# theOehrly/Formula-VAD

Measured on AMD Instinct MI355X. Metric: 48 kHz 480-sample VAD frames/sec whole node; max concurrent real-time streams, higher is better.
Workload: dtype f32

## Files before the change

### formula-vad_amd/csrc/fvad_vadm.hip

```cpp
#pragma clang fp contract(off)
#include <hip/hip_runtime.h>

#include "fvad_device.h"
#include "fvad_exact.h"
#include "fvad_internal.h"
#include "fvad_launch.h"
#include "fvad_staged.h"
#include "fvad_staged_dev.h"
#include "fvad_vadm_dev.h"

namespace fvad {

__device__ void vadm_stream(const StagedArgs &a, int m, int s, float *lt, size_t lts, bool final) {
  const int B = a.n_streams, C = a.n_channels, nb = a.n_bands;
  const int nt = ticks_of(a, s);
  const VadmConst &K = a.vadm.c[m];
  VadmState S = a.vadm.st[(size_t)m * B + s];
  float *st = a.vadm.buf + K.st_off + s, *rb = a.vadm.buf + K.r_off + s;
  VadmSeg *seg = a.vadm.seg + ((size_t)m * B + s) * a.vadm.seg_cap;
  const VadmEvLane ev = vadm_ev_lane(a.vadm, m, s);
  vadm_walk(S, K, st, rb, B, lt, lts, seg, a.vadm.seg_cap, ev, (unsigned long long)a.plan->nfft_b,
            a.vadm.bound_scale, a.vadm.defer_max, a.vadm.count, final, [&](auto &&window) {
              for (int t = 0; t < nt; t++)
                for (int w = 0, nw = a.out_win_flag[(size_t)t * B + s]; w < nw; w++) {
                  const size_t o = ((size_t)t * B + s) * a.wpt + w;
                  float min_v = 999, max_v = 0;
                  for (int c = 0; c < C; c++) {
                    const float v = a.out_band[(o * C + c) * nb + K.slot];
                    if (v < min_v) min_v = v;
                    if (v > max_v) max_v = v;
                  }
                  if ((long long)S.windows_done == a.vadm.negate_at) min_v = -min_v;
                  window(min_v, a.use_denoiser ? a.out_win_vad[o] : 0.0f, a.out_win_ratio[o]);
                }
            });
  a.vadm.st[(size_t)m * B + s] = S;
}

#ifndef FVAD_VP_BLOCK
#define FVAD_VP_BLOCK 8
#endif
constexpr int kVpG = 16, kVpS = 4, kVpMaxW = 48;
__device__ __forceinline__ double lt_fold(double acc, const float *lt, size_t lts, unsigned i0, unsigned i1, unsigned nw,
                                          double init, double scalar) {
  if (i0 >= i1) return acc;
  return lt_range<FVAD_VP_BLOCK>(acc, lt, lts, i0, i1, nw, init, scalar);
}
__global__ void __launch_bounds__(64) k_vadm_par(StagedArgs a) {
  __shared__ float wmin[kVpS][kVpMaxW], wvad[kVpS][kVpMaxW], wvr[kVpS][kVpMaxW];
  __shared__ float pv[kVpS][kVpMaxW];
  __shared__ double favg[kVpS][kVpG];
  __shared__ double rpre[kVpS];
  __shared__ int rnd[kVpS][4];
  __shared__ VadmState Ss[kVpS];
  const int B = a.n_streams, C = a.n_channels, nb = a.n_bands;
  const int g = threadIdx.x / kVpG, r = threadIdx.x % kVpG;
  const int s = blockIdx.x * kVpS + g;
  const bool sok = s < B && ticks_of(a, s) > 0;
  const int nt = sok ? ticks_of(a, s) : 0;
  const unsigned long long fft = (unsigned long long)a.plan->nfft_b;
  const int self = threadIdx.x;
  for (int m = 0; m < a.vadm.n; m++) {
    const VadmConst &K = a.vadm.c[m];
    float *lt = a.vadm.buf + K.lt_off + (size_t)(sok ? s : 0) * K.lt_pitch;
    const size_t lts = 1;
    int Kw = 0;
    for (int t0 = 0; t0 < nt; t0 += kVpG) {
      const int t = t0 + r;
      const int nwt = t < nt ? a.out_win_flag[(size_t)t * B + s] : 0;
      int pos = nwt;
#pragma unroll
      for (int d = 1; d < kVpG; d <<= 1) {
        const int up = __shfl(pos, self - d);
        if (r >= d) pos += up;
      }
      const int tot = __shfl(pos, g * kVpG + kVpG - 1);
      for (int w = 0; w < nwt; w++) {
        const int k = Kw + pos - nwt + w;
        if (k < kVpMaxW) {
          const size_t o = ((size_t)t * B + s) * a.wpt + w;
          float min_v = 999;
          for (int c = 0; c < C; c++) {
            const float v = a.out_band[(o * C + c) * nb + K.slot];
            if (v < min_v) min_v = v;
          }
          wmin[g][k] = min_v;
          wvad[g][k] = a.use_denoiser ? a.out_win_vad[o] : 0.0f;
          wvr[g][k] = a.out_win_ratio[o];
        }
      }
      Kw += tot;
    }
    if (r == 0) {
      Ss[g] = a.vadm.st[(size_t)m * B + (sok ? s : 0)];
      if (sok) {
        lt_resolve(Ss[g], K, lt, lts);
      } else if (s < B) {
        VadmState S2 = a.vadm.st[(size_t)m * B + s];
        if (S2.lt_defer) {
          lt_resolve(S2, K, a.vadm.buf + K.lt_off + (size_t)s * K.lt_pitch, 1);
          a.vadm.st[(size_t)m * B + s] = S2;
        }
      }
    }
    wave_sync();
    if (r == 0 && sok && a.vadm.negate_at >= 0) {
      const long long k = a.vadm.negate_at - (long long)Ss[g].windows_done;
      if (k >= 0 && k < Kw && k < kVpMaxW) wmin[g][k] = -wmin[g][k];
      wave_sync();
    }
    VadmState &S = Ss[g];
    float *st = a.vadm.buf + K.st_off + (sok ? s : 0), *rb = a.vadm.buf + K.r_off + (sok ? s : 0);
    VadmSeg *seg = a.vadm.seg + ((size_t)m * B + (sok ? s : 0)) * a.vadm.seg_cap;
    const VadmEvLane ev = vadm_ev_lane(a.vadm, m, sok ? s : 0);
    const bool forced = a.vadm.par_serial_every > 0 && s % a.vadm.par_serial_every == 0;
    const bool fast = sok && !forced && Kw <= kVpMaxW && K.n_lt > kVpMaxW && S.lt_count == (unsigned)K.n_lt &&
                      S.lt_pre_ok;
    const unsigned n = (unsigned)K.n_lt, wbase = S.lt_widx, nw0 = S.lt_nw;
    const double scalar = 1.0 / (double)n;
    if (r == 0) {
      rnd[g][0] = 0;
      rnd[g][1] = 0;
      rnd[g][2] = !sok ? 1 : (fast ? 0 : 2);
    }
    wave_sync();
    int j = 0, npush = 0;
    double pre = S.lt_pre;
    for (;;) {
      if (r == 0 && rnd[g][2] == 0) {
        while (j < Kw) {
          const unsigned long long index = S.windows_done * fft;
          const bool met = vadm_short(S, K, st, rb, B, wmin[g][j], wvr[g][j]);
          if (!met) break;
          S.windows_done++;
          vadm_fsm(S, K, index, met, wvad[g][j], wvr[g][j], seg, a.vadm.seg_cap, ev);
          j++;
        }
        if (j >= Kw) rnd[g][2] = 1;
        rnd[g][0] = j;
        rnd[g][1] = npush;
        for (int q = 0; q < kVpG && j + q < Kw; q++) pv[g][npush + q] = wmin[g][j + q];
        rpre[g] = pre;
      }
      wave_sync();
      const int state = rnd[g][2];
      if (__ballot(state == 0) == 0) break;
      if (state == 0) {
        const int j0 = rnd[g][0], np = rnd[g][1];
        if (j0 + r < Kw) {
          const unsigned k = (unsigned)(np + r);
          const unsigned nw = min(n, nw0 + k + 1);
          double P = rpre[g];
          unsigned w = (wbase + (unsigned)np) % n;
#pragma unroll 1
          for (int q = 0; q < r; q++) {
            P = (w + 1 == n) ? 0.0 : P + (double)pv[g][np + q] * scalar;
            w = (w + 1 == n) ? 0u : w + 1;
          }
          double acc = P + (double)pv[g][np + r] * scalar;
          if (wbase + k < n) {
            acc = lt_fold(acc, lt, lts, w + 1, n, nw, K.init, scalar);
          } else {
            acc = lt_fold(acc, lt, lts, w + 1, wbase, nw, K.init, scalar);
            for (unsigned i = wbase; i < n; i++) acc += (double)pv[g][i - wbase] * scalar;
          }
          favg[g][r] = acc;
        }
      }
      wave_sync();
      if (r == 0 && state == 0) {
        const int j0 = j;
        for (int q = 0; q < kVpG && j0 + q < Kw; q++) {
          const int jj = j0 + q;
          const unsigned long long index = S.windows_done * fft;
          bool met = false;
          if (q > 0) met = vadm_short(S, K, st, rb, B, wmin[g][jj], wvr[g][jj]);
          if (!met) {
            const unsigned w = S.lt_widx;
            S.lt_widx = (w + 1) % n;
            if (S.lt_nw < n) S.lt_nw++;
            pre = (w + 1 == n) ? 0.0 : pre + (double)wmin[g][jj] * scalar;
            S.lt_pre = pre;
            S.lt_last = favg[g][q];
            S.lt_has = 1;
            lt_neg_push(S, n, wmin[g][jj]);
            npush++;
          }
          S.windows_done++;
          vadm_fsm(S, K, index, met, wvad[g][jj], wvr[g][jj], seg, a.vadm.seg_cap, ev);
          j = jj + 1;
          if (met) break;
        }
      }
      wave_sync();
    }
    if (r == 0 && sok) {
      if (rnd[g][2] == 2) {
        vadm_stream(a, m, s, lt, lts, true);
      } else {
        unsigned w = wbase;
#pragma unroll 1
        for (int q = 0; q < npush; q++) {
          lt[(size_t)w * lts] = pv[g][q];
          w = (w + 1 == n) ? 0u : w + 1;
        }
        a.vadm.st[(size_t)m * B + s] = S;
      }
    }
    wave_sync();
  }
}

#ifndef FVAD_VADM_LANES
#define FVAD_VADM_LANES 64
#endif
constexpr int kVadmHbmLanes = FVAD_VADM_LANES;
__global__ void __launch_bounds__(64) k_vadm_hbm(StagedArgs a) {
  const int s = blockIdx.x * blockDim.x + threadIdx.x;
  if (s >= a.n_streams) return;
  const bool final = a.vadm.vfinal != 0;
  if (ticks_of(a, s) <= 0) {
    if (final)
      for (int m = 0; m < a.vadm.n; m++) {
        VadmState *p = a.vadm.st + (size_t)m * a.n_streams + s;
        if (p->lt_defer) {
          VadmState S = *p;
          lt_resolve(S, a.vadm.c[m], a.vadm.buf + a.vadm.c[m].lt_off + (size_t)s * a.vadm.c[m].lt_pitch, 1);
          *p = S;
        }
      }
    return;
  }
  for (int m = 0; m < a.vadm.n; m++)
    vadm_stream(a, m, s, a.vadm.buf + a.vadm.c[m].lt_off + (size_t)s * a.vadm.c[m].lt_pitch, 1, final);
}

hipError_t launch_vadm(const StagedArgs &a, hipStream_t stream, bool fast, bool *ran_par) {
  (void)hipGetLastError();
  bool par = fast && a.wmax <= kVpMaxW;
  for (int m = 0; m < a.vadm.n; m++) par = par && a.vadm.c[m].has_init && a.vadm.c[m].n_lt > kVpMaxW;
  if (ran_par) *ran_par = par;
  if (!par)
    FVAD_KERNEL_TRY(k_vadm_hbm, dim3((a.n_streams + kVadmHbmLanes - 1) / kVadmHbmLanes), dim3(kVadmHbmLanes), 0,
                    stream, a);
  else
    FVAD_KERNEL_TRY(k_vadm_par, dim3((a.n_streams + kVpS - 1) / kVpS), dim3(kVpS * kVpG), 0, stream, a);
  return hipSuccess;
}

constexpr int kEvThreads = 256;
__global__ void __launch_bounds__(kEvThreads) k_vadm_events(VadmEventArgs a) {
  __shared__ unsigned wsum[kEvThreads / 64];
  const int tid = threadIdx.x, wl = tid & 63, wave = tid >> 6;
  const unsigned long long wr0 = a.cursor[0];
  const unsigned long long used = wr0 - a.host_read;
  const unsigned long long room = used < a.ring_cap ? a.ring_cap - used : 0ull;
  const int chunk = a.chunk > 0 && a.chunk < kEvThreads ? a.chunk : kEvThreads;
  unsigned long long base = 0;
  for (int l0 = 0; l0 < a.n_lanes; l0 += chunk) {
    const int l = l0 + tid;
    const bool on = tid < chunk && l < a.n_lanes;
    const unsigned c = on ? min(a.count[l], (unsigned)a.ev_cap) : 0u;
    unsigned inc = c;
#pragma unroll
    for (int d = 1; d < 64; d <<= 1) {
      const unsigned up = __shfl_up(inc, d);
      if (wl >= d) inc += up;
    }
    if (wl == 63) wsum[wave] = inc;
    __syncthreads();
    unsigned before = 0, total = 0;
#pragma unroll
    for (int w = 0; w < kEvThreads / 64; w++) {
      const unsigned v = wsum[w];
      if (w < wave) before += v;
      total += v;
    }
    const unsigned long long first = base + before + (inc - c);
    for (unsigned j = 0; j < c; j++) {
      const unsigned long long pos = first + j;
      if (pos >= room) break;
      const VadmEvRec r = a.stage[(size_t)l * a.ev_cap + j];
      VadmEvent e;
      e.kind = r.kind;
      e.stream = l / a.n_machines;
      e.machine = l % a.n_machines;
      e.seq = r.seq;
      e.push = a.push;
      e.sample_from = r.sample_from;
      e.sample_to = r.sample_to;
      e.debug_rnn_vad = r.debug_rnn_vad;
      e.debug_avg_speech_vol_ratio = r.debug_avg_speech_vol_ratio;
      a.ring[(wr0 + pos) % a.ring_cap] = e;
    }
    if (c) a.count[l] = 0;
    base += total;
    __syncthreads();
  }
  if (tid == 0) {
    const unsigned long long written = base < room ? base : room;
    const unsigned long long lost = a.cursor[1] + (base - written);
    a.cursor[0] = wr0 + written;
    a.cursor[1] = lost;
    VadmEventHeader h;
    h.pass = a.pass;
    h.end = wr0 + written;
    h.lost = lost;
    h.n = base;
    *a.header = h;
  }
}

hipError_t launch_vadm_events(const VadmEventArgs &a, hipStream_t stream) {
  (void)hipGetLastError();
  FVAD_KERNEL_TRY(k_vadm_events, dim3(1), dim3(kEvThreads), 0, stream, a);
  return hipSuccess;
}

constexpr int kSelStreams = 4;
#ifndef FVAD_SEL_RING
#define FVAD_SEL_RING 8
#endif
constexpr int kSelRing = FVAD_SEL_RING;
struct SelRec {
  int T0, nv, Tk, offk, off0;
  float g0, xy0, yy0, gk, xyk, yyk;
};
__device__ __forceinline__ void sel_load(SelRec &r, const float *__restrict__ row, int k, bool on) {
  if (!on) return;
  r.T0 = __float_as_int(row[rec::kT0]);
  r.nv = __float_as_int(row[rec::kNValid]);
  r.g0 = row[rec::kG0];
  r.xy0 = row[rec::kXy0];
  r.yy0 = row[rec::kYy0];
  r.off0 = __float_as_int(row[rec::kOff0]);
  const float *q = row + rec::kK + min(k, 13) * rec::kKStride;
  r.Tk = __float_as_int(q[0]);
  r.gk = q[1];
  r.xyk = q[2];
  r.yyk = q[3];
  r.offk = __float_as_int(q[4]);
}

__global__ void __launch_bounds__(64) k_select(StagedArgs a) {
  const int lane = threadIdx.x, sl = lane >> 4, k = lane & 15;
  static_assert(kWorkSlots * kQueues <= 64, "one lane per counter");
  if (blockIdx.x == 0 && lane < kWorkSlots * kQueues) a.work[lane] = 0;
  const int s = blockIdx.x * kSelStreams + sl;
  const bool sok = s < a.n_streams;
  const int nf = sok ? ticks_of(a, s) * a.n_channels : 0;
  int nfw = nf;
#pragma unroll
  for (int d = 16; d < 64; d <<= 1) nfw = max(nfw, __shfl_xor(nfw, d));
  if (nfw <= 0) return;
  float *stp = a.state + (size_t)(sok ? s : 0) * st::kWords;
  int *istp = reinterpret_cast<int *>(stp);
  int last_period = sok ? istp[st::kLastPeriod] : 0;
  float last_gain = sok ? stp[st::kLastGain] : 0.0f;
  const float *rows = a.rec + (size_t)(sok ? s : 0) * a.V * rec::kSize;
  const int K = k + 2;
  auto step = [&](const SelRec &r, int v) {
    const bool on = v < nf;
    const int prev_period = last_period / 2;
    const float prev_gain = last_gain;
    bool pass = false;
    if (on && k < 14 && k < r.nv) {
      const int T1 = r.Tk;
      float cont;
      if (abs(T1 - prev_period) <= 1)
        cont = prev_gain;
      else if (abs(T1 - prev_period) <= 2 && 5 * K * K < r.T0)
        cont = .5f * prev_gain;
      else
        cont = 0;
      float thresh;
      {
        const float vv = .7f * r.g0 - cont;
        thresh = (.3f > vv) ? .3f : vv;
      }
      if (T1 < 3 * 30) {
        const float vv = .85f * r.g0 - cont;
        thresh = (.4f > vv) ? .4f : vv;
      } else if (T1 < 2 * 30) {
        const float vv = .9f * r.g0 - cont;
        thresh = (.5f > vv) ? .5f : vv;
      }
      pass = r.gk > thresh;
    }
    const unsigned seg = (unsigned)(__ballot(pass) >> (16 * sl)) & 0x3fffu;
    const int win = seg ? 31 - __clz(seg) : 0;
    const int src = 16 * sl + win;
    const float wxy = __shfl(r.xyk, src), wyy = __shfl(r.yyk, src), wg = __shfl(r.gk, src);
    const int wT = __shfl(r.Tk, src), woff = __shfl(r.offk, src);
    float best_xy = seg ? wxy : r.xy0, best_yy = seg ? wyy : r.yy0, gg = seg ? wg : r.g0;
    const int T = seg ? wT : r.T0, offset = seg ? woff : r.off0;
    if (!on) return;
    best_xy = (0 > best_xy) ? 0 : best_xy;
    float pg;
    if (best_yy <= best_xy)
      pg = 1.0f;
    else
      pg = best_xy / (best_yy + 1);
    if (pg > gg) pg = gg;
    int pi = 2 * T + offset;
    if (pi < kPitchMin) pi = kPitchMin;
    if (k == 0) a.pitch[(size_t)s * a.V + v] = pi;
    last_period = pi;
    last_gain = pg;
  };
  SelRec r[kSelRing];
#pragma unroll
  for (int u = 0; u < kSelRing - 1; u++) {
    r[u] = SelRec{};
    sel_load(r[u], rows + (size_t)u * rec::kSize, k, u < nf);
  }
  r[kSelRing - 1] = SelRec{};
  for (int v = 0; v < nfw; v += kSelRing) {
#pragma unroll
    for (int u = 0; u < kSelRing; u++) {
      if (v + u >= nfw) break;
      const int ls = (u + kSelRing - 1) % kSelRing;
      sel_load(r[ls], rows + (size_t)(v + u + kSelRing - 1) * rec::kSize, k, v + u + kSelRing - 1 < nf);
      step(r[u], v + u);
    }
  }
  if (sok && nf > 0 && k == 0) {
    istp[st::kLastPeriod] = last_period;
    stp[st::kLastGain] = last_gain;
  }
}

hipError_t launch_select(const StagedArgs &a, hipStream_t stream) {
  FVAD_KERNEL_TRY(k_select, dim3((a.n_streams + kSelStreams - 1) / kSelStreams), dim3(64), 0, stream, a);
  return hipSuccess;
}

}
```

Baseline: 45.27 million.

## Precompute per-candidate select terms ahead and cut k_select's serial dependency chain

Restructures k_select so the work that does not depend on the previous frame's pitch (pg, pi, threshold base/floor, live mask) is computed a few frames ahead in sel_prep. The serial step is reduced to one ballot plus two ds_bpermute lookups. Records are loaded with vector memcpy and clamped indices instead of predicated scalar loads. Pitch outputs are buffered per lane and written once per ring pass instead of one lane storing every frame. This shortens the loop-carried latency chain at the cost of more registers for the ring of prepared options.

```diff
diff --git a/formula-vad_amd/csrc/fvad_vadm.hip b/formula-vad_amd/csrc/fvad_vadm.hip
--- a/formula-vad_amd/csrc/fvad_vadm.hip
+++ b/formula-vad_amd/csrc/fvad_vadm.hip
@@ -321,29 +321,76 @@
 #ifndef FVAD_SEL_RING
 #define FVAD_SEL_RING 8
 #endif
+#ifndef FVAD_SEL_AHEAD
+#define FVAD_SEL_AHEAD 2
+#endif
 constexpr int kSelRing = FVAD_SEL_RING;
+constexpr int kSelAhead = FVAD_SEL_AHEAD;
+static_assert(kSelRing <= 16 && kSelAhead >= 1 && kSelAhead <= kSelRing - 2, "k_select's ring");
+typedef float SelF4 __attribute__((ext_vector_type(4)));
+typedef float SelF2 __attribute__((ext_vector_type(2)));
 struct SelRec {
-  int T0, nv, Tk, offk, off0;
-  float g0, xy0, yy0, gk, xyk, yyk;
+  SelF4 sh;
+  SelF2 sh2;
+  SelF4 c;
+  float coff;
 };
-__device__ __forceinline__ void sel_load(SelRec &r, const float *__restrict__ row, int k, bool on) {
-  if (!on) return;
-  r.T0 = __float_as_int(row[rec::kT0]);
-  r.nv = __float_as_int(row[rec::kNValid]);
-  r.g0 = row[rec::kG0];
-  r.xy0 = row[rec::kXy0];
-  r.yy0 = row[rec::kYy0];
-  r.off0 = __float_as_int(row[rec::kOff0]);
-  const float *q = row + rec::kK + min(k, 13) * rec::kKStride;
-  r.Tk = __float_as_int(q[0]);
-  r.gk = q[1];
-  r.xyk = q[2];
-  r.yyk = q[3];
-  r.offk = __float_as_int(q[4]);
+struct SelOpt {
+  int T1, pi;
+  float g1, base, floor, pg;
+  bool near2;
+  unsigned long long live;
+};
+static_assert(rec::kT0 == 0 && rec::kNValid == 1 && rec::kG0 == 2 && rec::kXy0 == 3 && rec::kYy0 == 4 &&
+                  rec::kOff0 == 5 && rec::kKStride == 5,
+              "sel_load's vectors");
+__device__ __forceinline__ SelRec sel_load(const float *__restrict__ row, int kk) {
+  SelRec r;
+  const float *q = row + rec::kK + kk * rec::kKStride;
+  __builtin_memcpy(&r.sh, row, sizeof r.sh);
+  __builtin_memcpy(&r.sh2, row + 4, sizeof r.sh2);
+  __builtin_memcpy(&r.c, q, sizeof r.c);
+  r.coff = q[4];
+  return r;
+}
+__device__ __forceinline__ SelOpt sel_prep(const SelRec &r, int j, bool on) {
+  SelOpt o;
+  const bool t0 = j == 0;
+  const int k = j - 1, K = k + 2;
+  const int T0 = __float_as_int(r.sh.x), nv = __float_as_int(r.sh.y), T1 = __float_as_int(r.c.x);
+  const float g0 = r.sh.z, g1 = r.c.y;
+  float best_xy = t0 ? r.sh.w : r.c.z;
+  const float best_yy = t0 ? r.sh2.x : r.c.w, gg = t0 ? g0 : g1;
+  const int T = t0 ? T0 : T1, offset = __float_as_int(t0 ? r.sh2.y : r.coff);
+  best_xy = (0 > best_xy) ? 0 : best_xy;
+  float pg;
+  if (best_yy <= best_xy)
+    pg = 1.0f;
+  else
+    pg = best_xy / (best_yy + 1);
+  if (pg > gg) pg = gg;
+  int pi = 2 * T + offset;
+  if (pi < kPitchMin) pi = kPitchMin;
+  o.pi = pi;
+  o.pg = pg;
+  o.T1 = T1;
+  o.g1 = g1;
+  o.near2 = 5 * K * K < T0;
+  o.base = .7f * g0;
+  o.floor = .3f;
+  if (T1 < 3 * 30) {
+    o.base = .85f * g0;
+    o.floor = .4f;
+  } else if (T1 < 2 * 30) {
+    o.base = .9f * g0;
+    o.floor = .5f;
+  }
+  o.live = __ballot(on && j >= 1 && j < 15 && k < nv);
+  return o;
 }
 
 __global__ void __launch_bounds__(64) k_select(StagedArgs a) {
-  const int lane = threadIdx.x, sl = lane >> 4, k = lane & 15;
+  const int lane = threadIdx.x, sl = lane >> 4, j = lane & 15;
   static_assert(kWorkSlots * kQueues <= 64, "one lane per counter");
   if (blockIdx.x == 0 && lane < kWorkSlots * kQueues) a.work[lane] = 0;
   const int s = blockIdx.x * kSelStreams + sl;
@@ -358,73 +405,50 @@
   int last_period = sok ? istp[st::kLastPeriod] : 0;
   float last_gain = sok ? stp[st::kLastGain] : 0.0f;
   const float *rows = a.rec + (size_t)(sok ? s : 0) * a.V * rec::kSize;
-  const int K = k + 2;
-  auto step = [&](const SelRec &r, int v) {
+  const int kk = min(max(j - 1, 0), 13);
+  const int flast = max(nf - 1, 0);
+  const unsigned long long t0s = 0x0001000100010001ull;
+  int keep = 0;
+  auto load = [&](int f) { return sel_load(rows + (size_t)min(f, flast) * rec::kSize, kk); };
+  auto step = [&](const SelOpt &o, int v, int u) {
     const bool on = v < nf;
     const int prev_period = last_period / 2;
     const float prev_gain = last_gain;
-    bool pass = false;
-    if (on && k < 14 && k < r.nv) {
-      const int T1 = r.Tk;
-      float cont;
-      if (abs(T1 - prev_period) <= 1)
-        cont = prev_gain;
-      else if (abs(T1 - prev_period) <= 2 && 5 * K * K < r.T0)
-        cont = .5f * prev_gain;
-      else
-        cont = 0;
-      float thresh;
-      {
-        const float vv = .7f * r.g0 - cont;
-        thresh = (.3f > vv) ? .3f : vv;
-      }
-      if (T1 < 3 * 30) {
-        const float vv = .85f * r.g0 - cont;
-        thresh = (.4f > vv) ? .4f : vv;
-      } else if (T1 < 2 * 30) {
-        const float vv = .9f * r.g0 - cont;
-        thresh = (.5f > vv) ? .5f : vv;
-      }
-      pass = r.gk > thresh;
-    }
-    const unsigned seg = (unsigned)(__ballot(pass) >> (16 * sl)) & 0x3fffu;
-    const int win = seg ? 31 - __clz(seg) : 0;
-    const int src = 16 * sl + win;
-    const float wxy = __shfl(r.xyk, src), wyy = __shfl(r.yyk, src), wg = __shfl(r.gk, src);
-    const int wT = __shfl(r.Tk, src), woff = __shfl(r.offk, src);
-    float best_xy = seg ? wxy : r.xy0, best_yy = seg ? wyy : r.yy0, gg = seg ? wg : r.g0;
-    const int T = seg ? wT : r.T0, offset = seg ? woff : r.off0;
-    if (!on) return;
-    best_xy = (0 > best_xy) ? 0 : best_xy;
-    float pg;
-    if (best_yy <= best_xy)
-      pg = 1.0f;
+    float cont;
+    if (abs(o.T1 - prev_period) <= 1)
+      cont = prev_gain;
+    else if (abs(o.T1 - prev_period) <= 2 && o.near2)
+      cont = .5f * prev_gain;
     else
-      pg = best_xy / (best_yy + 1);
-    if (pg > gg) pg = gg;
-    int pi = 2 * T + offset;
-    if (pi < kPitchMin) pi = kPitchMin;
-    if (k == 0) a.pitch[(size_t)s * a.V + v] = pi;
-    last_period = pi;
-    last_gain = pg;
+      cont = 0;
+    const float vv = o.base - cont;
+    const float thresh = (o.floor > vv) ? o.floor : vv;
+    const unsigned long long pass = (__ballot(o.g1 > thresh) & o.live) | t0s;
+    const unsigned seg = (unsigned)(pass >> (16 * sl)) & 0x7fffu;
+    const int addr = (16 * sl + 31 - __clz(seg)) << 2;
+    const int pi = __builtin_amdgcn_ds_bpermute(addr, o.pi);
+    const float pg = __int_as_float(__builtin_amdgcn_ds_bpermute(addr, __float_as_int(o.pg)));
+    last_period = on ? pi : last_period;
+    last_gain = on ? pg : last_gain;
+    keep = (j == u) ? pi : keep;
   };
   SelRec r[kSelRing];
-#pragma unroll
-  for (int u = 0; u < kSelRing - 1; u++) {
-    r[u] = SelRec{};
-    sel_load(r[u], rows + (size_t)u * rec::kSize, k, u < nf);
-  }
-  r[kSelRing - 1] = SelRec{};
+  SelOpt o[kSelRing];
+#pragma unroll
+  for (int u = 0; u < kSelRing - 1; u++) r[u] = load(u);
+#pragma unroll
+  for (int u = 0; u < kSelAhead; u++) o[u] = sel_prep(r[u], j, u < nf);
   for (int v = 0; v < nfw; v += kSelRing) {
 #pragma unroll
     for (int u = 0; u < kSelRing; u++) {
-      if (v + u >= nfw) break;
-      const int ls = (u + kSelRing - 1) % kSelRing;
-      sel_load(r[ls], rows + (size_t)(v + u + kSelRing - 1) * rec::kSize, k, v + u + kSelRing - 1 < nf);
-      step(r[u], v + u);
-    }
-  }
-  if (sok && nf > 0 && k == 0) {
+      r[(u + kSelRing - 1) % kSelRing] = load(v + u + kSelRing - 1);
+      const int up = (u + kSelAhead) % kSelRing;
+      o[up] = sel_prep(r[up], j, v + u + kSelAhead < nf);
+      step(o[u], v + u, u);
+    }
+    if (sok && j < kSelRing && v + j < nf) a.pitch[(size_t)s * a.V + v + j] = keep;
+  }
+  if (sok && nf > 0 && j == 0) {
     istp[st::kLastPeriod] = last_period;
     stp[st::kLastGain] = last_gain;
   }
```

After: 45.13 million. No clear change (-0.3%).
